# AI4REALNET/network-distributed-q-learning

Hardware: NVIDIA B200
Metric: switch_agent_decisions_per_sec (higher is better)
Workload: dtype f64

## Files before the change

### network-distributed-q-learning_b200/csrc/sfl_api.cu

```cuda
#include <stdio.h>
#include <stdlib.h>
#include <string.h>
#include <new>
#include <vector>

#include "sfl_core.cuh"

using namespace sfl;

static thread_local char g_err[512] = "";
static int fail(int code, const char *fmt, const char *detail = "") {
  snprintf(g_err, sizeof(g_err), fmt, detail);
  return code;
}

#ifndef SFL_HOST_EMUL
#include <cuda_runtime.h>
#define CU(call)                                                               \
  do {                                                                         \
    cudaError_t e_ = (call);                                                   \
    if (e_ != cudaSuccess) return fail(SFL_E_CUDA, "CUDA: %s", cudaGetErrorString(e_)); \
  } while (0)
#define CK(call)                                                               \
  do {                                                                         \
// ... 900 lines not shown
  k_shared_apply<<<c->sm_count * 8, 256, 0, (cudaStream_t)stream>>>(src, dst, d, cn, n);
  CU(cudaGetLastError());
#else
  (void)stream;
  for (size_t i = 0; i < n; i++) {
    double v = src[i];
    if (cn[i]) { v += (double)d[i] / 16777216.0 / (double)cn[i]; d[i] = 0; cn[i] = 0; }
    dst[i] = v;
  }
#endif
  return SFL_OK;
}

int sfl_shared_q_apply(void *ctx, void *stream) {
  Ctx *c = (Ctx *)ctx;
  if (!c || !c->bound) return fail(SFL_E_STATE, "sfl_bind first%s");
  DeviceGuard dg(c->device);
  if (!c->cfg.shared_q) return fail(SFL_E_STATE, "context was not created in shared-table mode%s");
  return shared_apply(c, (const double *)c->bufs.shared_q, (double *)c->bufs.shared_q, (long long *)c->bufs.shared_d, (int *)c->bufs.shared_c, stream);
}

int sfl_shared_q_apply_to(void *ctx, const void *q_src, void *q_dst, void *d, void *cnt, void *stream) {
  Ctx *c = (Ctx *)ctx;
  if (!c || !q_src || !q_dst || !d || !cnt) return fail(SFL_E_ARG, "null argument%s");
  if (!c->cfg.shared_q) return fail(SFL_E_STATE, "context was not created in shared-table mode%s");
  DeviceGuard dg(c->device);
  return shared_apply(c, (const double *)q_src, (double *)q_dst, (long long *)d, (int *)cnt, stream);
}

int sfl_total_decisions(void *ctx, uint64_t *decisions, uint64_t *ticks, void *stream) {
  Ctx *c = (Ctx *)ctx;
  if (!c || !c->bound) return fail(SFL_E_STATE, "sfl_bind first%s");
  DeviceGuard dg(c->device);
  unsigned long long out[2] = {0, 0};
#ifndef SFL_HOST_EMUL
  CK(dev_zero(c->sum_buf, 16, stream));
  k_sum<<<c->sm_count, 256, 0, (cudaStream_t)stream>>>((const sfl_env_counters *)c->bufs.counters, c->cfg.n_envs, (unsigned long long *)c->sum_buf);
  CU(cudaGetLastError());
  CK(d2h(out, c->sum_buf, 16, stream));
#else
  const sfl_env_counters *cn = (const sfl_env_counters *)c->bufs.counters;
  for (int i = 0; i < c->cfg.n_envs; i++) { out[0] += cn[i].decisions; out[1] += cn[i].ticks; }
#endif
  if (decisions) *decisions = out[0];
  if (ticks) *ticks = out[1];
  return SFL_OK;
}

int sfl_export_q(void *ctx, int env, uint32_t *keys_host, double *vals_host, int cap_rows, int *n_rows, void *stream) {
  Ctx *c = (Ctx *)ctx;
  if (!c || !c->bound) return fail(SFL_E_STATE, "sfl_bind first%s");
  DeviceGuard dg(c->device);
  if (c->cfg.eval_q) return fail(SFL_E_STATE, "an evaluation context (eval_q) keeps no per-environment tables%s");
  if (env < 0 || env >= c->cfg.n_envs || !n_rows) return fail(SFL_E_ARG, "bad env / n_rows%s");
  const Layout &L = c->L;
  size_t n = (size_t)L.q_cap * L.q_stride;
  std::vector<double> img(n);
  CK(d2h(img.data(), (char *)c->bufs.state + (size_t)env * L.env_stride + L.off_q, n * 8, stream));
  int rows = 0;
  for (int i = 0; i < L.q_cap; i++) {
    unsigned long long k;
    memcpy(&k, &img[(size_t)i * L.q_stride], 8);
    if (!k) continue;
    if (rows < cap_rows && keys_host && vals_host) {
      keys_host[rows] = (uint32_t)(k - 1);
      for (int a = 0; a < L.a_max; a++) vals_host[(size_t)rows * L.a_max + a] = img[(size_t)i * L.q_stride + 1 + a];
    }
    rows++;
  }
  *n_rows = rows;
  return rows > cap_rows && keys_host ? fail(SFL_E_NOMEM, "export buffer too small%s") : SFL_OK;
}

int sfl_import_q(void *ctx, int env, const uint32_t *keys_host, const double *vals_host, int n_rows, void *stream) {
  Ctx *c = (Ctx *)ctx;
  if (!c || !c->bound) return fail(SFL_E_STATE, "sfl_bind first%s");
  DeviceGuard dg(c->device);
  if (c->cfg.eval_q) return fail(SFL_E_STATE, "an evaluation context (eval_q) keeps no per-environment tables: use sfl_set_eval_table%s");
  if (env < 0 || env >= c->cfg.n_envs || n_rows < 0 || n_rows >= c->cfg.q_cap) return fail(SFL_E_ARG, "bad env / n_rows%s");
  const Layout &L = c->L;
  std::vector<double> img;
  int q_rows = q_image(L, keys_host, vals_host, n_rows, img);
  char *base = (char *)c->bufs.state + (size_t)env * L.env_stride;
  CK(h2d(base + L.off_q, img.data(), img.size() * 8, stream));
  CK(h2d(base + offsetof(EnvHdr, q_rows), &q_rows, 4, stream));
#ifndef SFL_HOST_EMUL
  CU(cudaStreamSynchronize((cudaStream_t)stream));
#endif
  return SFL_OK;
}

int sfl_set_eval_table(void *ctx, const uint32_t *keys_host, const double *vals_host, int n_rows, void *stream) {
  Ctx *c = (Ctx *)ctx;
  if (!c || !c->bound) return fail(SFL_E_STATE, "sfl_bind first%s");
  if (!c->cfg.eval_q) return fail(SFL_E_STATE, "the context was not created as an evaluation context (eval_q)%s");
  if (n_rows < 0 || (n_rows && (!keys_host || !vals_host))) return fail(SFL_E_ARG, "bad keys / values / n_rows%s");
  if (n_rows >= c->cfg.q_cap) {
    char detail[96];
    snprintf(detail, sizeof(detail), "%d rows, q_cap is %d", n_rows, c->cfg.q_cap);
    return fail(SFL_E_NOMEM, "the evaluation table needs q_cap above its row count (a power of two; an empty slot ends every probe): %s", detail);
  }
  DeviceGuard dg(c->device);
  std::vector<double> img;
  q_image(c->L, keys_host, vals_host, n_rows, img);
  CK(h2d(c->bufs.eval_q, img.data(), img.size() * 8, stream));
#ifndef SFL_HOST_EMUL
  CU(cudaStreamSynchronize((cudaStream_t)stream));
#endif
  return SFL_OK;
}

}
```

### network-distributed-q-learning_b200/csrc/sfl_core.cuh

```cuda
#pragma once
#include <stdint.h>
#include "switchfl_b200.h"

#if defined(__CUDACC__) && !defined(SFL_HOST_EMUL)
#define SFL_DEV 1
#define SFL_FN __device__ __forceinline__
#define SFL_NI __device__ __forceinline__
#define SFL_RARE __device__ __noinline__
#define SFL_NU _Pragma("unroll 1")
#define SFL_U4 _Pragma("unroll 4")
#define SFL_UA _Pragma("unroll")
#else
#define SFL_DEV 0
#include <math.h>
#include <string.h>
#define SFL_FN inline
#define SFL_NI inline
#define SFL_RARE inline
#define SFL_NU
#define SFL_U4
#define SFL_UA
struct int4 { int x, y, z, w; };
struct int2 { int x, y; };
static inline int4 make_int4(int x, int y, int z, int w) { int4 r = {x, y, z, w}; return r; }
// ... 47 lines not shown
};
SFL_FN int popc64(unsigned long long v) { return __builtin_popcountll(v); }
SFL_FN int ffs64(unsigned long long v) { return __builtin_ffsll((long long)v) - 1; }
SFL_FN int popc32(unsigned v) { return __builtin_popcount(v); }
SFL_FN double dmul(double a, double b) { volatile double r = a * b; return r; }
SFL_FN double dadd(double a, double b) { volatile double r = a + b; return r; }
SFL_FN double dfma(double a, double b, double c) { return fma(a, b, c); }
SFL_FN unsigned long long mulhi64(unsigned long long a, unsigned long long b) { return (unsigned long long)(((unsigned __int128)a * b) >> 64); }
template <class T> SFL_FN T ldg(const T *p) { return *p; }
#endif

template <int NW> struct TSet {
  static_assert(NW == 1 || NW == 2, "one or two words of trains");
  unsigned long long w[NW];
  SFL_FN void clear() { w[0] = 0ull; if (NW > 1) w[NW - 1] = 0ull; }
  SFL_FN void or_ballot(unsigned b, int base) {
    if (NW == 1) { w[0] |= (unsigned long long)b << base; return; }
    const unsigned long long v = (unsigned long long)b << (base & 63);
    if (base < 64) w[0] |= v; else w[NW - 1] |= v;
  }
  SFL_FN unsigned long long test(int t) const {
    if (NW == 1) return (w[0] >> t) & 1ull;
    return ((t < 64 ? w[0] : w[NW - 1]) >> (t & 63)) & 1ull;
  }
  SFL_FN int any() const { return NW == 1 ? w[0] != 0ull : (w[0] | w[NW - 1]) != 0ull; }
  SFL_FN int popc() const { return NW == 1 ? popc64(w[0]) : popc64(w[0]) + popc64(w[NW - 1]); }
  SFL_FN int pop() {
    if (NW == 1 || w[0]) { const int t = ffs64(w[0]); w[0] &= w[0] - 1; return t; }
    const int t = 64 + ffs64(w[NW - 1]); w[NW - 1] &= w[NW - 1] - 1; return t;
  }
  SFL_FN int all(int T) const {
    if (NW == 1) return w[0] == (T >= 64 ? ~0ull : ((1ull << T) - 1ull));
    return w[0] == ~0ull && w[NW - 1] == (T >= 128 ? ~0ull : ((1ull << (T - 64)) - 1ull));
  }
  SFL_FN TSet andnot(const TSet &o) const { TSet r; r.w[0] = w[0] & ~o.w[0]; if (NW > 1) r.w[NW - 1] = w[NW - 1] & ~o.w[NW - 1]; return r; }
  SFL_FN int operator==(const TSet &o) const { return NW == 1 ? w[0] == o.w[0] : (w[0] == o.w[0]) & (w[NW - 1] == o.w[NW - 1]); }
};

template <class T> struct RO {
  const T *p;
  SFL_FN T operator[](size_t i) const { return ldg(p + i); }
};

struct DevMap {
  int H, W, Hp, Wp, S, NP, NA, T, NT, max_episode_steps, a_max, pad0;
  RO<uint16_t> move;
  RO<int16_t> cell_switch;
  RO<int4> sw;
  RO<int4> port;
  RO<int4> pexit;
  RO<int4> act;
  RO<int4> train0;
  RO<int4> train1;
  RO<int> init_delay;
  RO<int> dist;
  RO<int8_t> qinit;
};

struct Layout {
  int T, S, NP, NT, a_max, q_cap, q_stride, pend_cap;
  unsigned off_tra, off_trb, off_pend, off_sem, off_rewards, off_sws, off_q;
  unsigned off_rng;
  unsigned long long env_stride;
};

struct EnvHdr {
  int elapsed, episode, step_counter, num_malf;
  int terminated, truncated, need_reset, halted;
  int err, q_rows, pending_fin, cur_dec;
  int act_cursor, ev_cursor, n_dec_logged, n_tick_logged;
  int n_ep_logged, q_init_on, aborted, cur_train;
  unsigned long long active_mask, malf_prev_mask, at_dest_mask, done_mask;
  unsigned long long decisions, ticks, train_ticks;
  double cum_reward;
  int last_next_sw;
  int eps_tag;
  unsigned eps_z, eps_w;
  unsigned long long forced_stops, stop_actions, arrived_trains;
  int dec_t, dec_go;
  unsigned long long ph[6], ph_t0;
};

struct SwS { int ninter, pad; double eps_pow; };
enum { HM_ACTIVE = 0, HM_MALF = 1, HM_DEST = 2, HM_DONE = 3 };

struct RunArgs {
  int mode, max_ticks, n_envs, trace_sem;
  int dec_cap, tick_cap, ep_cap, act_cap, ev_cap, max_steps, q_init_on, phase_clock;
  unsigned hot_bytes, env_smem, tail_hot, pad2;
  char *state;
  const sfl_hparams *hp;
  sfl_env_counters *counters;
  sfl_dec_rec *trace_dec; sfl_tick_rec *trace_tick; int4 *trace_sem_buf;
  sfl_ep_rec *ep_log; int *ep_delay;
  sfl_step_rec *step_out;
  double *sq_q; long long *sq_d; int *sq_c;
  const int8_t *replay_act; const int *replay_ev;
  const double *eval_q;
};

struct KArgs { DevMap m; Layout L; RunArgs ra; };
#define SFL_K const KArgs &K
#define c_m (K.m)
#define c_L (K.L)
#define c_ra (K.ra)

#if SFL_DEV
extern __shared__ __align__(16) char g_smem[];
typedef unsigned hot_t;
SFL_FN char *hot_ptr(hot_t o) { return g_smem + o; }
#else
typedef char *hot_t;
SFL_FN char *hot_ptr(hot_t o) { return o; }
#endif

template <bool TH, bool SQ_ = false> struct EnvT {
  static const bool SQ = SQ_;
  static const bool EVQ = false;
  static const bool HOT_TAIL = TH;
  static const int NW = 1;
  const KArgs *kp;
  hot_t hot;
  char *gb;
  SFL_FN EnvHdr *h() const { return (EnvHdr *)hot_ptr(hot); }
  SFL_FN int4 *tra() const { return (int4 *)(hot_ptr(hot) + kp->L.off_tra); }
  SFL_FN int4 *trb() const { return (int4 *)(hot_ptr(hot) + kp->L.off_trb); }
  SFL_FN char *tail() const { return TH ? hot_ptr(hot) : gb; }
  SFL_FN int2 *pend() const { return (int2 *)(tail() + kp->L.off_pend); }
  SFL_FN int4 *sem() const { return (int4 *)(tail() + kp->L.off_sem); }
  SFL_FN int *rewards() const { return (int *)(tail() + kp->L.off_rewards); }
  SFL_FN SwS *sws() const { return (SwS *)(tail() + kp->L.off_sws); }
  SFL_FN double *q() const { return (double *)(gb + kp->L.off_q); }
  hot_t own;
  SFL_FN uint8_t *own_ptr() const { return (uint8_t *)hot_ptr(own); }
  SFL_FN int owner(int p) const { return TH ? sem()[p].z : (int)(int8_t)own_ptr()[p]; }
  SFL_FN void sem_put(int p, int4 r) const { sem()[p] = r; if (!TH) own_ptr()[p] = (uint8_t)r.z; }
  SFL_FN void sem_drop(int p) const { sem()[p].z = -1; if (!TH) own_ptr()[p] = 0xFFu; }
  SFL_FN int stop_tick(int t) const { return trb()[t].w; }
  SFL_FN unsigned long long &hw0(int m) const {
    EnvHdr *x = h();
    return m == HM_ACTIVE ? x->active_mask : m == HM_MALF ? x->malf_prev_mask : m == HM_DEST ? x->at_dest_mask : x->done_mask;
  }
  SFL_FN unsigned long long *hw1(int m) const { return (unsigned long long *)(hot_ptr(hot) + sizeof(EnvHdr)) + m; }
};
template <bool TH, bool SQ_ = false> struct EnvW : EnvT<TH, SQ_> { static const int NW = 2; };
template <class Base> struct EnvEval : Base { static const bool EVQ = true; };
template <bool TH, bool SQ, int NW, bool EVQ = false> struct EnvOf { typedef EnvT<TH, SQ> type; };
template <bool TH, bool SQ> struct EnvOf<TH, SQ, 2, false> { typedef EnvW<TH, SQ> type; };
template <bool TH, int NW> struct EnvOf<TH, false, NW, true> { typedef EnvEval<typename EnvOf<TH, false, NW>::type> type; };

template <class Env> SFL_FN TSet<Env::NW> tset(const Env &e, int m) {
  TSet<Env::NW> s; s.w[0] = e.hw0(m); if (Env::NW > 1) s.w[Env::NW - 1] = *e.hw1(m); return s;
}
template <class Env> SFL_FN void tset_put(const Env &e, int m, const TSet<Env::NW> &s) { e.hw0(m) = s.w[0]; if (Env::NW > 1) *e.hw1(m) = s.w[Env::NW - 1]; }
template <class Env> SFL_FN int tset_any(const Env &e, int m) { return Env::NW == 1 ? e.hw0(m) != 0ull : (e.hw0(m) | *e.hw1(m)) != 0ull; }
template <class Env> SFL_FN int tset_pop(const Env &e, int m) { TSet<Env::NW> s = tset(e, m); const int t = s.pop(); tset_put(e, m, s); return t; }
template <class Env> SFL_FN void tset_add(const Env &e, int m, int t) {
  if (Env::NW > 1 && t >= 64) *e.hw1(m) |= 1ull << (t & 63); else e.hw0(m) |= 1ull << t;
}



struct Scratch {
  const KArgs *kp;
  hot_t base;
  SFL_FN int4 *tmp() const { return (int4 *)hot_ptr(base); }
// ... 193 lines not shown
  int n = 0, pos = SFL_MT_N;
  const unsigned rng = (unsigned)hi - (unsigned)lo;
  SFL_NU
  for (int tick = 1; hit_below && tick <= steps; tick++) {
    SFL_NU
    for (int t = 0; t < T; t++) {
      const unsigned a = mt_next(key, out, pos, g), b = mt_next(key, out, pos, g);
      if ((((unsigned long long)(a >> 5) << 26) | (b >> 6)) >= hit_below) continue;
      const int dur = lo + (int)mt_masked(key, out, pos, g, rng) + 1;
      if (g.gl == 0 && n < ev_cap) { ev[3 * n] = tick; ev[3 * n + 1] = t; ev[3 * n + 2] = dur; }
      n++;
    }
  }
  if (g.gl == 0 && n < ev_cap) ev[3 * n] = -1;
  return n;
}

struct Mv { int cell, dir, valid; };
SFL_FN unsigned mv_entry(SFL_K, int cell, int dir) { return c_m.move[(size_t)cell * 4 + dir]; }
SFL_FN int mv_valid(unsigned e, int action) { return (e >> (3 * action)) & 1; }
SFL_FN Mv mv_apply(SFL_K, unsigned e, int action, int cell) {
  unsigned f = (e >> (3 * action)) & 7u;
  int nd = (int)(f >> 1);
  int delta = (nd & 1) ? (2 - nd) : (nd - 1) * c_m.Wp;
  Mv r;
  r.cell = (e & 0x8000u) ? cell + delta : cell;
  r.dir = nd; r.valid = (int)(f & 1u);
  return r;
}
SFL_FN Mv check_action(SFL_K, int action, int cell, int dir) { return mv_apply(K, mv_entry(K, cell, dir), action, cell); }

SFL_FN int is_moving(int a) { return a >= A_LEFT && a <= A_RIGHT; }

#define SFL_NO_STOP (-0x7FFFFFFF - 1)
SFL_FN int t0_eff(int t0, int stop_tick) { return t0 > stop_tick ? t0 : stop_tick; }
template <class Env>
SFL_FN int tr_state(Env e, int t) { return (e.tra()[t].y >> 8) & 0xFF; }
template <class Env>
SFL_FN int rule_port(Env e, int port, int me, int now, int blocking_type) {
  int4 r;
  int stamp;
  if (Env::HOT_TAIL) {
    r = e.sem()[port];
    if (r.z < 0 || r.z == me) return 0;
    stamp = e.stop_tick(r.z);
  } else {
    const int holder = e.owner(port);
    if (holder < 0 || holder == me) return 0;
    r = e.sem()[port];
    stamp = e.stop_tick(holder);
  }
  if (r.x > now || t0_eff(r.x, stamp) + r.y < now) return 0;
  if (r.w == blocking_type) return 1;
  return tr_state(e, r.z) == ST_MALF;
}
template <class Env>
SFL_FN int port_blocked(Env e, int next_port, int out_port, int me, int now) {
  if (next_port >= 0) {
    if (rule_port(e, next_port, me, now, SEM_OUT)) return 1;
    return rule_port(e, out_port, me, now, SEM_IN);
  }
  return rule_port(e, out_port, me, now, SEM_OUT);
}

template <class Env>
SFL_RARE void q_insert(SFL_K, Env e, const Hp hp, unsigned key, double *row) {
  *(unsigned long long *)row = (unsigned long long)key + 1ull;
  e.h()->q_rows++;
  unsigned per_port = (unsigned)(c_L.NT * 48);
  int port = (int)(key / per_port);
  int A = c_m.sw[c_m.port[port].w].y;
  double dq = hp->default_q;
  SFL_NU
  for (int a = 0; a < A; a++) row[1 + a] = dq;
  if (c_ra.q_init_on) {
    unsigned rem = key - (unsigned)port * per_port;
    int tgt = (int)(rem / 48u), semb = (int)((rem % 48u) / 3u);
    int qi = c_m.qinit[port * c_L.NT + tgt];
    if (qi >= 0 && semb != 0) row[1 + (qi & 15)] = (qi & 16) ? 1000.0 : 500.0;
  }
}

template <class Env>
SFL_NI double *q_row(SFL_K, Env e, const Hp hp, unsigned key) {
  if (Env::SQ) return c_ra.sq_q + (size_t)key * c_L.a_max;
  unsigned mask = (unsigned)c_L.q_cap - 1u;
  unsigned i = (key * 2654435761u) >> 7;
  SFL_NU
  for (int probe = 0; probe < c_L.q_cap; probe++) {
    i &= mask;
    double *row = e.q() + (size_t)i * c_L.q_stride;
    unsigned long long k = *(unsigned long long *)row;
    if (k == (unsigned long long)key + 1ull) return row + 1;
    if (k == 0ull) {
      if (e.h()->q_rows >= c_L.q_cap - 1) break;
      q_insert(K, e, hp, key, row);
      return row + 1;
    }
    i++;
  }
  e.h()->err |= SFL_ERR_Q_FULL;
  return e.q() + 1;
}

#if SFL_DEV
SFL_FN void shared_add(long long *d, int *c, long long v) { atomicAdd((unsigned long long *)d, (unsigned long long)v); atomicAdd(c, 1); }
#else
SFL_FN void shared_add(long long *d, int *c, long long v) { *d += v; *c += 1; }
#endif

SFL_FN double lr_pow(double rate, int n) {
  double r = 1.0, b = rate;
  SFL_NU
  for (; n > 0; n >>= 1) { if (n & 1) r = dmul(r, b); b = dmul(b, b); }
  return r;
}

SFL_FN double td_value(double q, double lr, double reward, double gamma, double mq, int bootstrap) {
  const double one_m = dadd(1.0, -lr);
  return bootstrap ? dadd(dmul(one_m, q), dmul(lr, dadd(reward, dmul(gamma, mq)))) : dadd(dmul(one_m, q), dmul(lr, reward));
}

template <class Env>
SFL_NI void q_update(SFL_K, Env e, const Hp hp, unsigned key, int action, double reward,
                     const double *next_row, int prev_sw, int next_sw) {
  double *row = q_row(K, e, hp, key);
  double lr = hp->lr;
  if (hp->lr_decay_rate != 1.0) lr = dmul(lr, lr_pow(hp->lr_decay_rate, e.sws()[prev_sw].ninter));
  const double q = row[action];
  double mq = 0.0;
  if (next_sw != prev_sw && next_row) {
    int A = c_m.sw[next_sw].y;
    mq = next_row[0];
    SFL_NU
    for (int a = 1; a < A; a++) { const double v = next_row[a]; mq = v > mq ? v : mq; }
  }
  const double nq = td_value(q, lr, reward, hp->gamma, mq, next_sw != prev_sw);
  if (Env::SQ) {
    const size_t i = (size_t)key * c_L.a_max + action;
    shared_add(c_ra.sq_d + i, c_ra.sq_c + i, (long long)llrint((nq - q) * 16777216.0));
    return;
  }
  row[action] = nq;
}

template <class Row> SFL_FN int max_action_of(const Row row, int A, int mask) {
  int best = 0, b2 = -1;
  double bv = row[0], b2v = 0.0;
  if (mask & 1) { b2 = 0; b2v = bv; }
  SFL_NU
  for (int a = 1; a < A; a++) {
    const double v = row[a];
    if (v > bv) { bv = v; best = a; }
    if (((mask >> a) & 1) && (b2 < 0 || v > b2v)) { b2v = v; b2 = a; }
  }
  return ((mask >> best) & 1) ? best : b2;
}
SFL_FN int max_action(const double *row, int A, int mask) { return max_action_of(row, A, mask); }

SFL_FN int eval_action(SFL_K, unsigned key, int A, int mask) {
  const unsigned qmask = (unsigned)c_L.q_cap - 1u;
  const unsigned long long want = (unsigned long long)key + 1ull;
  unsigned i = (key * 2654435761u) >> 7;
  SFL_NU
  for (int probe = 0; probe < c_L.q_cap; probe++) {
    i &= qmask;
    const double *row = c_ra.eval_q + (size_t)i * c_L.q_stride;
    const unsigned long long k = ldg((const unsigned long long *)row);
    if (k == want) { RO<double> r; r.p = row + 1; return max_action_of(r, A, mask); }
    if (k == 0ull) break;
    i++;
  }
  return ffs64((unsigned long long)((unsigned)mask & ((1u << A) - 1u)));
}

template <class Env>
SFL_FN void sem_delete_owned(SFL_K, Env e, int port, int h) {
  int4 sw = c_m.sw[c_m.port[port].w];
  SFL_NU
  for (int k = 0; k < sw.x; k++) {
    int p = sw.z + k;
    if (e.owner(p) == h) e.sem_drop(p);
  }
}

template <class Env>
SFL_FN void transition_semaphore(SFL_K, Env e, int source, int out_port, int target, int h, int now, int st, int old_next, int old_prev) {
  if (st != ST_MALF) {
    sem_delete_owned(K, e, old_next, h);
    if (old_prev >= 0) sem_delete_owned(K, e, old_prev, h);
  }
  if (Env::HOT_TAIL) {
    int4 r = e.sem()[out_port];
    if (r.z < 0) e.sem()[out_port] = make_int4(now, 3, h, SEM_OUT);
    else if (r.w == SEM_OUT || r.x > now) e.sem()[out_port] = make_int4(now, 3, h, r.w);
    int d_ot = c_m.port[out_port].y;
    r = e.sem()[target];
    if (r.z < 0) e.sem()[target] = make_int4(now, d_ot + 1, h, SEM_IN);
    else if (r.w == SEM_IN || r.x > now) e.sem()[target] = make_int4(now, d_ot + 1, h, r.w);
    int unique = c_m.port[target].z;
    if (unique >= 0) {
      int4 up = c_m.port[unique];
      int far_port = up.x;
      if (unique != source && unique != out_port && unique != target) {
        r = e.sem()[unique];
        if (r.z < 0 || r.w == SEM_OUT || r.x > now) e.sem()[unique] = make_int4(now, d_ot + 1, h, SEM_OUT);
      }
      r = e.sem()[unique];
      if (r.z < 0 || r.x > now) e.sem()[unique] = make_int4(now, d_ot, h, SEM_OUT);
      if (far_port != source && far_port != out_port && far_port != unique) {
        r = e.sem()[far_port];
        if (r.z < 0 || r.w == SEM_IN || r.x > now) e.sem()[far_port] = make_int4(now, d_ot + up.y + 1, h, SEM_IN);
      }
    }
    if (target != source && target != out_port) {
      r = e.sem()[target];
      if (r.z < 0 || r.w == SEM_OUT || r.x > now) e.sem()[target] = make_int4(now, d_ot + 1, h, SEM_OUT);
    }
  } else {
    int4 r;
    if (e.owner(out_port) < 0) e.sem_put(out_port, make_int4(now, 3, h, SEM_OUT));
    else { r = e.sem()[out_port]; if (r.w == SEM_OUT || r.x > now) e.sem_put(out_port, make_int4(now, 3, h, r.w)); }
    int d_ot = c_m.port[out_port].y;
    if (e.owner(target) < 0) e.sem_put(target, make_int4(now, d_ot + 1, h, SEM_IN));
    else { r = e.sem()[target]; if (r.w == SEM_IN || r.x > now) e.sem_put(target, make_int4(now, d_ot + 1, h, r.w)); }
    int unique = c_m.port[target].z;
    if (unique >= 0) {
      int4 up = c_m.port[unique];
      int far_port = up.x;
      if (unique != source && unique != out_port && unique != target) {
        r = e.sem()[unique];
        if (e.owner(unique) < 0 || r.w == SEM_OUT || r.x > now) e.sem_put(unique, make_int4(now, d_ot + 1, h, SEM_OUT));
      }
      r = e.sem()[unique];
      if (e.owner(unique) < 0 || r.x > now) e.sem_put(unique, make_int4(now, d_ot, h, SEM_OUT));
      if (far_port != source && far_port != out_port && far_port != unique) {
        r = e.sem()[far_port];
        if (e.owner(far_port) < 0 || r.w == SEM_IN || r.x > now) e.sem_put(far_port, make_int4(now, d_ot + up.y + 1, h, SEM_IN));
      }
    }
    if (target != source && target != out_port) {
      r = e.sem()[target];
      if (e.owner(target) < 0 || r.w == SEM_OUT || r.x > now) e.sem_put(target, make_int4(now, d_ot + 1, h, SEM_OUT));
    }
  }
}

template <class Env>
SFL_FN int delay_at(SFL_K, Env e, int tgt_index, int cell, int dir, int now, int la) {
  int d = c_m.dist[((size_t)tgt_index * (c_m.Hp * c_m.Wp) + cell) * 4 + dir];
  if (d >= SFL_INF_DIST) { e.h()->err |= SFL_ERR_INF_DISTANCE; d = 0; }
  return now - la + d;
}

template <int KIND, class Env>
SFL_FN void finish_decision(SFL_K, Env e, const Hp hp, int env_id) {
  const bool TRACE = KIND == K_FULL;
  const int mode = run_mode<KIND>(K);
  EnvHdr *h = e.h();
  SFL_PHASE_START(h);
  if (mode == SFL_MODE_LEARN || mode == SFL_MODE_REPLAY) {
    TSet<Env::NW> fresh = tset(e, HM_DONE).andnot(tset(e, HM_DEST));
    SFL_NU
    while (fresh.any()) {
      int t = fresh.pop();
      tset_add(e, HM_DEST, t);
      int4 b = e.trb()[t];
      int n = (b.y >> 16) & 0xFF;
      SFL_NU
      for (int i = 0; i < n; i++) {
        int2 pe = e.pend()[t * c_L.pend_cap + i];
        q_update(K, e, hp, (unsigned)pe.x, (pe.y >> 24) & 15, 1000.0, nullptr, (pe.y >> 12) & 0xFFF, -1);
      }
      b.y &= 0xFFFF;
      e.trb()[t] = b;
    }
    SwS *ss = e.sws() + h->pending_fin;
    ss->ninter++;
    ss->eps_pow = dmul(ss->eps_pow, hp->epsilon_decay_rate);
  }
  h->pending_fin = -1;
  SFL_PHASE_MARK(h, PH_UPDATE);
  if (h->step_counter > c_ra.max_steps) h->truncated = 1;
  if (TRACE) {
    if (c_ra.trace_dec && h->cur_dec >= 0 && h->cur_dec < c_ra.dec_cap) {
      sfl_dec_rec *rec = c_ra.trace_dec + (size_t)env_id * c_ra.dec_cap + h->cur_dec;
      rec->arrived = h->done_mask; rec->arrived_hi = Env::NW > 1 ? *e.hw1(HM_DONE) : 0ull;
      rec->done = h->terminated | (h->truncated << 1);
      if (c_ra.trace_sem_buf) {
        int4 *dst = c_ra.trace_sem_buf + ((size_t)env_id * c_ra.dec_cap + h->cur_dec) * c_L.NP;
        SFL_NU
        for (int p = 0; p < c_L.NP; p++) {
          int4 r = e.sem()[p];
          if (r.z >= 0) r.x = t0_eff(r.x, e.stop_tick(r.z));
          r.y += r.x; dst[p] = r;
        }
      }
    }
    h->cur_dec = -1;
  }
}

template <int G, class Env>
SFL_FN int observe_bits(SFL_K, Env e, const Grp<G> &g, const int on, const int t) {
  const int now = e.h()->elapsed;
  const int s = on ? (e.trb()[t].y & 0xFFFF) : 0;
  const int4 sw = c_m.sw[s];
  unsigned bits = 0;
  SFL_UA
  for (int base = 0; base < 8; base += G) {
    const int j = base + g.gl;
    int b = 0;
    if (on && j < 8 && (j & 3) < sw.x) {
      const int port = sw.z + (j & 3);
      b = (j & 4) ? rule_port(e, port, t, now, SEM_IN) : rule_port(e, c_m.port[port].x, t, now, SEM_OUT);
    }
    bits |= (g.ballot(b) & 0xFFu) << base;
  }
  return (int)(~(bits | (bits >> 4)) & ((1u << sw.x) - 1u));
}

struct Obs { int s, P, A, p0, a0, cur, semb, mask, ok; unsigned key; };
template <class Env>
SFL_FN Obs observe(SFL_K, Env e, int t, int now, const int4 ta, const int4 tb, const int semb_pre = -1) {
  Obs ob;
  ob.s = tb.y & 0xFFFF;
  const int4 sw = c_m.sw[ob.s];
  ob.P = sw.x; ob.A = sw.y; ob.p0 = sw.z; ob.a0 = sw.w;
  const int4 tr0 = c_m.train0[t], tr1 = c_m.train1[t];
  const int my_port = (int)((unsigned)ta.w >> 16);
  const int dist_now = c_m.dist[((size_t)tr0.w * (c_m.Hp * c_m.Wp) + ta.x) * 4 + (ta.y & 0xFF)];
  int semb = semb_pre;
  if (semb_pre < 0) {
    semb = 0;
    SFL_NU
    for (int k = 0; k < ob.P; k++)
      if (!port_blocked(e, c_m.port[ob.p0 + k].x, ob.p0 + k, t, now)) semb |= 1 << k;
  }
  ob.semb = semb;
  ob.cur = my_port - ob.p0;
  ob.ok = ob.cur >= 0 && ob.cur < ob.P;
  ob.key = 0u; ob.mask = 0;
  if (!ob.ok) return ob;
  int delay = now - tr1.y + dist_now;
  if (dist_now >= SFL_INF_DIST) { e.h()->err |= SFL_ERR_INF_DISTANCE; delay = now - tr1.y; }
  int level = delay <= 0 ? 0 : (delay <= (tr1.y - tr1.x) * 20 ? 1 : 2);
  ob.key = (((unsigned)(ob.p0 + ob.cur) * c_L.NT + tr0.w) * 16u + semb) * 3u + level;
  const int4 px = c_m.pexit[ob.p0 + ob.cur];
  int mask = 1 << (ob.A - 1);
  {
    int ex[3] = {px.y, px.z, px.w};
#if SFL_DEV
#pragma unroll
#endif
    for (int i = 0; i < 3; i++) if (i < px.x && ((semb >> ((ex[i] >> 4) & 3)) & 1)) mask |= 1 << (ex[i] & 15);
  }
  ob.mask = mask;
  return ob;
}

template <int KIND, class Env>
SFL_FN void decide(SFL_K, Env e, const Hp hp, int env_id, int t, const int semb_pre = -1) {
  const bool TRACE = KIND == K_FULL;
  const int mode = run_mode<KIND>(K);
  EnvHdr *h = e.h();
  const int now = h->elapsed;
  SFL_PHASE_START(h);
  int4 ta = e.tra()[t], tb = e.trb()[t];
  const int learning = mode == SFL_MODE_LEARN || mode == SFL_MODE_REPLAY;
  const int s_early = tb.y & 0xFFFF;
  const int reward_in = e.rewards()[s_early * c_L.T + t];
  double eps_pow = 1.0;
  int ninter = 0;
  if (mode == SFL_MODE_LEARN) {
    eps_pow = e.sws()[s_early].eps_pow;
    if (KIND == K_FULL && c_L.off_rng) ninter = e.sws()[s_early].ninter;
  }
  int2 pend0 = make_int2(0, -1);
  if (learning && ((tb.y >> 16) & 0xFF)) pend0 = e.pend()[t * c_L.pend_cap];
  const Obs ob = observe(K, e, t, now, ta, tb, semb_pre);
  if (!ob.ok) {
    h->err |= SFL_ERR_NO_TRAIN_AT_SWITCH; h->aborted++; h->truncated = 1;
    return;
  }
  const int s = ob.s, A = ob.A, p0 = ob.p0, a0 = ob.a0, cur = ob.cur, mask = ob.mask;
  const unsigned key = ob.key;
  const int4 tr0 = c_m.train0[t], tr1 = c_m.train1[t];
  const int pos = ta.x, dir = ta.y & 0xFF, st = (ta.y >> 8) & 0xFF;
  const int my_port = (int)((unsigned)ta.w >> 16);
  SFL_PHASE_MARK(h, PH_OBSERVE);
  double *my_row = nullptr;
  int action = -1;
  if (mode == SFL_MODE_REPLAY || mode == SFL_MODE_STEP) {
    if (mode == SFL_MODE_STEP) h->act_cursor = 0;
    int exploited = 0;
    if (h->act_cursor >= c_ra.act_cap) { h->err |= SFL_ERR_REPLAY_UNDERRUN; action = A - 1; }
    else {
      action = c_ra.replay_act[(size_t)env_id * c_ra.act_cap + h->act_cursor++];
      if (mode == SFL_MODE_REPLAY && action >= 0 && (action & 0x40)) { exploited = 1; action &= 0x3F; }
    }
    if (action < 0 || action >= A) { h->err |= SFL_ERR_BAD_ACTION; action = A - 1; }
    if (exploited) {
      my_row = q_row(K, e, hp, key);
      if (max_action(my_row, A, mask) != action) h->err |= SFL_ERR_REPLAY_DIVERGED;
    }
  } else if (KIND == K_FULL && mode == SFL_MODE_LEARN && c_L.off_rng) {
    Pcg *gp = (Pcg *)(hot_ptr(e.hot) + c_L.off_rng);
    Pcg g = *gp;
    if (eps_explore(pcg_double(g), hp->epsilon, hp->epsilon_decay_rate, ninter, eps_pow)) action = pcg_explore_action(g, mask);
    *gp = g;
  } else if (mode == SFL_MODE_LEARN) {
    double eps = dmul(hp->epsilon, eps_pow);
    const int pair = h->step_counter >> 1;
    unsigned ux, uy;
    if ((h->step_counter & 1) && h->eps_tag == pair) { ux = h->eps_z; uy = h->eps_w; }
    else {
      const U4 u = philox4x32((unsigned)pair, (unsigned)(hp->episode_base + h->episode), 0x5F1u, 0u, (unsigned)hp->seed, (unsigned)(hp->seed >> 32));
      h->eps_tag = pair; h->eps_z = u.z; h->eps_w = u.w;
      if (h->step_counter & 1) { ux = u.z; uy = u.w; } else { ux = u.x; uy = u.y; }
    }
    double u01 = ((double)ux + 0.5) * (1.0 / 4294967296.0);
    if (u01 < eps) {
      int pick = (int)(((unsigned long long)uy * (unsigned)popc32((unsigned)mask)) >> 32);
      unsigned mm = (unsigned)mask;
      SFL_NU
      for (; pick > 0; pick--) mm &= mm - 1;
      action = ffs64(mm);
    }
  }
  if (action < 0) {
    if (Env::EVQ) action = eval_action(K, key, A, mask);
    else {
      my_row = q_row(K, e, hp, key);
      action = max_action(my_row, A, mask);
    }
  }
  SFL_PHASE_MARK(h, PH_ACT);
  int moving = 0, move2 = A_STOP, in_port = my_port, out_port = my_port;
  if (action != A - 1) {
    int4 ac = c_m.act[a0 + action];
    if (ac.x == cur) { moving = 1; move2 = ac.z; in_port = p0 + ac.x; out_port = p0 + ac.y; }
  }
  int next_switch = s, next_port = -1;
  if (moving) {
    int4 op = c_m.port[out_port];
    next_port = op.x;
    int old_prev = (tb.x & 0xFFFF) == 0xFFFF ? -1 : (tb.x & 0xFFFF);
    transition_semaphore(K, e, in_port, out_port, next_port, t, now, st, my_port, old_prev);
    tb.x = (out_port & 0xFFFF) | (in_port << 16);
    ta.w = (ta.w & 0xFFFF) | (next_port << 16);
    next_switch = c_m.port[next_port].w;
  }
  unsigned plan = (unsigned)ta.z & 0xFFFFu;
  int pl = ta.z >> 16;
  if (moving && pl > 0) { plan = (plan & 0xFu) | ((unsigned)move2 << 4); pl = 2; }
  else if (!moving) {
    if (pl >= SFL_PLAN_CAP) { h->err |= SFL_ERR_PLAN_FULL; pl = SFL_PLAN_CAP - 1; }
    plan = ((plan << 4) | A_STOP) & 0xFFFFu; pl++;
  } else { plan = A_FWD | ((unsigned)move2 << 4); pl = 2; }
  ta.z = (int)plan | (pl << 16);
  e.tra()[t] = ta;
  int all_blocked = 1;
  if ((plan & 0xFu) == A_STOP) {
    if (moving) all_blocked = port_blocked(e, next_port, out_port, t, now);
    else all_blocked = (mask == (1 << (A - 1)));
  }
  int cell = pos, d2 = dir;
  {
    unsigned pp = plan;
    SFL_NU
    for (int i = 0; i < pl; i++, pp >>= 4) {
      int a = pp & 0xF;
      if (a != A_STOP) { Mv c = check_action(K, a, cell, d2); cell = c.cell; d2 = c.dir; }
    }
  }
  int curr = delay_at(K, e, tr0.w, cell, d2, now, tr1.y);
  int reward_out = tb.z - curr;
  if (!all_blocked && (plan & 0xFu) == A_STOP) reward_out -= 1300;
  e.rewards()[next_switch * c_L.T + t] = reward_out;
  tb.z = curr;
  h->step_counter++;
  SFL_PHASE_MARK(h, PH_APPLY);
  if (learning) {
    int n = (tb.y >> 16) & 0xFF;
    int2 *pend = e.pend() + t * c_L.pend_cap;
    int hit = -1, same = -1;
    SFL_NU
    for (int i = 0; i < n; i++) {
      int nsw = (i ? pend[i].y : pend0.y) & 0xFFF;
      if (nsw == s && hit < 0) hit = i;
    }
    if (hit >= 0) {
      int2 pe = hit ? pend[hit] : pend0;
      const int prev_sw = (pe.y >> 12) & 0xFFF;
      if (prev_sw != s && !my_row) my_row = q_row(K, e, hp, key);
      q_update(K, e, hp, (unsigned)pe.x, (pe.y >> 24) & 15, (double)reward_in, my_row, prev_sw, s);
      SFL_NU
      for (int j = hit; j + 1 < n; j++) pend[j] = pend[j + 1];
      n--;
    }
    int meta = next_switch | (s << 12) | (action << 24);
    SFL_NU
    for (int i = 0; i < n; i++) if ((pend[i].y & 0xFFF) == next_switch) same = i;
    if (same >= 0) pend[same] = make_int2((int)key, meta);
    else if (n >= c_L.pend_cap) h->err |= SFL_ERR_PEND_FULL;
    else { pend[n] = make_int2((int)key, meta); n++; }
    tb.y = (tb.y & 0xFFFF) | (n << 16);
  }
  e.trb()[t] = tb;
  SFL_PHASE_MARK(h, PH_UPDATE);
  h->cum_reward += (double)reward_in;
  if (TRACE) {
    if (c_ra.trace_dec) {
      h->cur_dec = h->n_dec_logged;
      if (h->n_dec_logged < c_ra.dec_cap) {
        sfl_dec_rec *rec = c_ra.trace_dec + (size_t)env_id * c_ra.dec_cap + h->n_dec_logged;
        rec->ep = h->episode; rec->tick = now; rec->sw = s; rec->train = t; rec->key = key; rec->mask = mask;
        rec->action = action; rec->next_sw = next_switch; rec->reward = reward_in; rec->done = 0; rec->arrived = 0;
        rec->arrived_hi = 0;
      }
      h->n_dec_logged++;
    }
  }
  if (TRACE) h->last_next_sw = next_switch;
  h->decisions++;
  if (mask == (1 << (A - 1))) h->forced_stops++;
  if (action == A - 1) h->stop_actions++;
  h->pending_fin = s;
}

template <int G, class Env>
SFL_RARE void env_reset(SFL_K, Env e, const Grp<G> &g, int on) {
  EnvHdr *h = e.h();
  const int T = on ? c_L.T : 0, NP = on ? c_L.NP : 0;
  SFL_NU
  for (int t = g.gl; t < T; t += G) {
    int4 tr0 = c_m.train0[t], tr1 = c_m.train1[t];
    e.tra()[t] = make_int4(-1, tr0.y | (ST_WAITING << 8) | (0 << 16) | (A_NONE << 24), 0, (int)((unsigned)tr1.z << 16));
    int4 b = e.trb()[t];
    e.trb()[t] = make_int4(b.x, 0xFFFF, c_m.init_delay[t], SFL_NO_STOP);
  }
  SFL_NU
  for (int p = g.gl; p < NP; p += G) e.sem_put(p, make_int4(0, 0, -1, 0));
  SFL_NU
  for (int i = g.gl; i < c_L.S * T; i += G) e.rewards()[i] = 0;
  g.sync();
  if (on && g.gl == 0) {
    SFL_NU
    for (int t = 0; t < T; t++) {
      int4 tr1 = c_m.train1[t];
      e.sem_put(tr1.z, make_int4(tr1.x - 2, tr1.w + 2, t, SEM_IN));
    }
    h->elapsed = 0; h->step_counter = 0; h->num_malf = 0; h->terminated = 0; h->truncated = 0; h->need_reset = 0;
    h->pending_fin = -1; h->cur_dec = -1; h->ev_cursor = 0; h->active_mask = 0; h->malf_prev_mask = 0; h->at_dest_mask = 0;
    h->eps_tag = -1;
    h->done_mask = 0; h->cum_reward = 0.0;
    if (Env::NW > 1) { SFL_UA for (int m = 0; m < 4; m++) *e.hw1(m) = 0ull; }
  }
  g.sync();
}

template <int NW> struct TickRegs {
  int elapsed, ended, rng_blk;
  TSet<NW> active, done;
  unsigned ticks, train_ticks;
};

SFL_FN int malf_stage2(const Hp hp, int now, int t) {
  const U4 u = philox4x32((unsigned)now, (unsigned)t, 0xA11Eu, 0u, (unsigned)hp->seed, (unsigned)(hp->seed >> 32));
  if (u.x >= hp->malf_thr2) return 0;
  return hp->malf_min + (int)(((unsigned long long)u.y * (unsigned)(hp->malf_max - hp->malf_min + 1)) >> 32) + 1;
}

template <int G, int KIND, bool ONE, class Env>
SFL_FN void env_tick(SFL_K, Env e, Scratch sc, const Hp hp, int env_id, const Grp<G> &g, TickRegs<Env::NW> &R, const int live) {
  const bool TRACE = KIND == K_FULL;
  EnvHdr *h = e.h();
  const int Tw = c_L.T;
  const int T = live ? Tw : 0;
  const int now = R.elapsed + 1;
  const int replay_ev = KIND != K_LEARN && c_ra.replay_ev != 0;
  const unsigned thr = live ? hp->malf_threshold : 0u;
  if (replay_ev) {
    SFL_NU
    for (int t = g.gl; t < T; t += G) sc.inj()[t] = 0;
    g.sync();
    if (live && g.gl == 0) {
      const int *ev = c_ra.replay_ev + (size_t)env_id * c_ra.ev_cap * 3;
      int c = h->ev_cursor;
// ... 402 lines not shown
```

Measured before the change: 425.1 million.

## Cache Q-table slot indices in pending updates to skip hash re-probing

Pending TD updates now store the Q-table slot index, tagged with a flag bit, in place of the raw key whenever the slot is known. The later update can then address the row directly instead of re-running the hash probe. The first two pending entries are prefetched with a single vector load, the hit's Q value is read early, and hit-removal and same-switch search are merged into one compaction pass. Importing a Q table now converts tagged entries back to keys on the host, because a rebuilt table invalidates the stored slots. This adds some host-side transfers on import.

```diff
diff --git a/network-distributed-q-learning_b200/csrc/sfl_api.cu b/network-distributed-q-learning_b200/csrc/sfl_api.cu
--- a/network-distributed-q-learning_b200/csrc/sfl_api.cu
+++ b/network-distributed-q-learning_b200/csrc/sfl_api.cu
@@ -1006,6 +1006,23 @@
   std::vector<double> img;
   int q_rows = q_image(L, keys_host, vals_host, n_rows, img);
   char *base = (char *)c->bufs.state + (size_t)env * L.env_stride;
+  std::vector<int4> trb(L.T);
+  std::vector<int2> pend((size_t)L.T * L.pend_cap);
+  CK(d2h(trb.data(), base + L.off_trb, trb.size() * sizeof(int4), stream));
+  CK(d2h(pend.data(), base + L.off_pend, pend.size() * sizeof(int2), stream));
+  int untagged = 0;
+  for (int t = 0; t < L.T; t++) {
+    const int n = (trb[t].y >> 16) & 0xFF;
+    for (int i = 0; i < n; i++) {
+      int2 &pe = pend[(size_t)t * L.pend_cap + i];
+      if (!(pe.y & SFL_PEND_SLOT)) continue;
+      unsigned long long k = 0;
+      CK(d2h(&k, base + L.off_q + (size_t)pe.x * L.q_stride * 8, 8, stream));
+      pe.x = (int)(unsigned)(k - 1ull); pe.y &= ~SFL_PEND_SLOT;
+      untagged++;
+    }
+  }
+  if (untagged) CK(h2d(base + L.off_pend, pend.data(), pend.size() * sizeof(int2), stream));
   CK(h2d(base + L.off_q, img.data(), img.size() * 8, stream));
   CK(h2d(base + offsetof(EnvHdr, q_rows), &q_rows, 4, stream));
 #ifndef SFL_HOST_EMUL
diff --git a/network-distributed-q-learning_b200/csrc/sfl_core.cuh b/network-distributed-q-learning_b200/csrc/sfl_core.cuh
--- a/network-distributed-q-learning_b200/csrc/sfl_core.cuh
+++ b/network-distributed-q-learning_b200/csrc/sfl_core.cuh
@@ -153,6 +153,7 @@
 };
 
 struct SwS { int ninter, pad; double eps_pow; };
+#define SFL_PEND_SLOT (1 << 28)
 enum { HM_ACTIVE = 0, HM_MALF = 1, HM_DEST = 2, HM_DONE = 3 };
 
 struct RunArgs {
@@ -512,7 +513,8 @@
 }
 
 template <class Env>
-SFL_NI double *q_row(SFL_K, Env e, const Hp hp, unsigned key) {
+SFL_NI double *q_row(SFL_K, Env e, const Hp hp, unsigned key, int &slot) {
+  slot = -1;
   if (Env::SQ) return c_ra.sq_q + (size_t)key * c_L.a_max;
   unsigned mask = (unsigned)c_L.q_cap - 1u;
   unsigned i = (key * 2654435761u) >> 7;
@@ -521,16 +523,25 @@
     i &= mask;
     double *row = e.q() + (size_t)i * c_L.q_stride;
     unsigned long long k = *(unsigned long long *)row;
-    if (k == (unsigned long long)key + 1ull) return row + 1;
+    if (k == (unsigned long long)key + 1ull) { slot = (int)i; return row + 1; }
     if (k == 0ull) {
       if (e.h()->q_rows >= c_L.q_cap - 1) break;
       q_insert(K, e, hp, key, row);
+      slot = (int)i;
       return row + 1;
     }
     i++;
   }
   e.h()->err |= SFL_ERR_Q_FULL;
   return e.q() + 1;
+}
+template <class Env>
+SFL_NI double *q_row(SFL_K, Env e, const Hp hp, unsigned key) { int slot; return q_row(K, e, hp, key, slot); }
+template <class Env>
+SFL_FN double *q_slot(SFL_K, Env e, int slot) { return e.q() + (size_t)slot * c_L.q_stride + 1; }
+template <class Env>
+SFL_NI double *pend_row(SFL_K, Env e, const Hp hp, int2 pe) {
+  return !Env::SQ && (pe.y & SFL_PEND_SLOT) ? q_slot(K, e, pe.x) : q_row(K, e, hp, (unsigned)pe.x);
 }
 
 #if SFL_DEV
@@ -552,12 +563,10 @@
 }
 
 template <class Env>
-SFL_NI void q_update(SFL_K, Env e, const Hp hp, unsigned key, int action, double reward,
+SFL_NI void q_update(SFL_K, Env e, const Hp hp, double *row, unsigned key, int action, double q, double reward,
                      const double *next_row, int prev_sw, int next_sw) {
-  double *row = q_row(K, e, hp, key);
   double lr = hp->lr;
   if (hp->lr_decay_rate != 1.0) lr = dmul(lr, lr_pow(hp->lr_decay_rate, e.sws()[prev_sw].ninter));
-  const double q = row[action];
   double mq = 0.0;
   if (next_sw != prev_sw && next_row) {
     int A = c_m.sw[next_sw].y;
@@ -699,8 +708,10 @@
       int n = (b.y >> 16) & 0xFF;
       SFL_NU
       for (int i = 0; i < n; i++) {
-        int2 pe = e.pend()[t * c_L.pend_cap + i];
-        q_update(K, e, hp, (unsigned)pe.x, (pe.y >> 24) & 15, 1000.0, nullptr, (pe.y >> 12) & 0xFFF, -1);
+        const int2 pe = e.pend()[t * c_L.pend_cap + i];
+        const int a = (pe.y >> 24) & 15;
+        double *row = pend_row(K, e, hp, pe);
+        q_update(K, e, hp, row, (unsigned)pe.x, a, row[a], 1000.0, nullptr, (pe.y >> 12) & 0xFFF, -1);
       }
       b.y &= 0xFFFF;
       e.trb()[t] = b;
@@ -806,8 +817,13 @@
     eps_pow = e.sws()[s_early].eps_pow;
     if (KIND == K_FULL && c_L.off_rng) ninter = e.sws()[s_early].ninter;
   }
-  int2 pend0 = make_int2(0, -1);
-  if (learning && ((tb.y >> 16) & 0xFF)) pend0 = e.pend()[t * c_L.pend_cap];
+  const int n_pend = learning ? (tb.y >> 16) & 0xFF : 0;
+  int2 *pend = e.pend() + t * c_L.pend_cap;
+  int2 pend0 = make_int2(0, -1), pend1 = make_int2(0, -1);
+  if (n_pend) {
+    if (c_L.pend_cap & 1) { pend0 = pend[0]; if (n_pend > 1) pend1 = pend[1]; }
+    else { const int4 v = *(const int4 *)pend; pend0 = make_int2(v.x, v.y); pend1 = make_int2(v.z, v.w); }
+  }
   const Obs ob = observe(K, e, t, now, ta, tb, semb_pre);
   if (!ob.ok) {
     h->err |= SFL_ERR_NO_TRAIN_AT_SWITCH; h->aborted++; h->truncated = 1;
@@ -820,6 +836,7 @@
   const int my_port = (int)((unsigned)ta.w >> 16);
   SFL_PHASE_MARK(h, PH_OBSERVE);
   double *my_row = nullptr;
+  int my_slot = -1;
   int action = -1;
   if (mode == SFL_MODE_REPLAY || mode == SFL_MODE_STEP) {
     if (mode == SFL_MODE_STEP) h->act_cursor = 0;
@@ -831,7 +848,7 @@
     }
     if (action < 0 || action >= A) { h->err |= SFL_ERR_BAD_ACTION; action = A - 1; }
     if (exploited) {
-      my_row = q_row(K, e, hp, key);
+      my_row = q_row(K, e, hp, key, my_slot);
       if (max_action(my_row, A, mask) != action) h->err |= SFL_ERR_REPLAY_DIVERGED;
     }
   } else if (KIND == K_FULL && mode == SFL_MODE_LEARN && c_L.off_rng) {
@@ -861,8 +878,17 @@
   if (action < 0) {
     if (Env::EVQ) action = eval_action(K, key, A, mask);
     else {
-      my_row = q_row(K, e, hp, key);
+      my_row = q_row(K, e, hp, key, my_slot);
       action = max_action(my_row, A, mask);
+    }
+  }
+  double q_hit = 0.0;
+  int q_hit_ok = 0;
+  if (!Env::SQ && n_pend && my_row) {
+    const int2 pe = (pend0.y & 0xFFF) == s ? pend0 : pend1;
+    if (((pend0.y & 0xFFF) == s || (n_pend > 1 && (pend1.y & 0xFFF) == s)) && (pe.y & SFL_PEND_SLOT)) {
+      q_hit = q_slot(K, e, pe.x)[(pe.y >> 24) & 15];
+      q_hit_ok = 1;
     }
   }
   SFL_PHASE_MARK(h, PH_ACT);
@@ -912,29 +938,34 @@
   h->step_counter++;
   SFL_PHASE_MARK(h, PH_APPLY);
   if (learning) {
-    int n = (tb.y >> 16) & 0xFF;
-    int2 *pend = e.pend() + t * c_L.pend_cap;
-    int hit = -1, same = -1;
+    int hit = -1, same = -1, n = 0;
+    int2 hit_e = make_int2(0, 0);
     SFL_NU
-    for (int i = 0; i < n; i++) {
-      int nsw = (i ? pend[i].y : pend0.y) & 0xFFF;
-      if (nsw == s && hit < 0) hit = i;
+    for (int i = 0; i < n_pend; i++) {
+      int2 pe;
+      if (i == 0) pe = pend0;
+      else if (i == 1) pe = pend1;
+      else pe = pend[i];
+      if (hit < 0 && (pe.y & 0xFFF) == s) { hit = i; hit_e = pe; continue; }
+      if ((pe.y & 0xFFF) == next_switch) same = n;
+      if (n != i) pend[n] = pe;
+      n++;
     }
     if (hit >= 0) {
-      int2 pe = hit ? pend[hit] : pend0;
-      const int prev_sw = (pe.y >> 12) & 0xFFF;
-      if (prev_sw != s && !my_row) my_row = q_row(K, e, hp, key);
-      q_update(K, e, hp, (unsigned)pe.x, (pe.y >> 24) & 15, (double)reward_in, my_row, prev_sw, s);
-      SFL_NU
-      for (int j = hit; j + 1 < n; j++) pend[j] = pend[j + 1];
-      n--;
-    }
-    int meta = next_switch | (s << 12) | (action << 24);
-    SFL_NU
-    for (int i = 0; i < n; i++) if ((pend[i].y & 0xFFF) == next_switch) same = i;
-    if (same >= 0) pend[same] = make_int2((int)key, meta);
+      const int prev_sw = (hit_e.y >> 12) & 0xFFF, a = (hit_e.y >> 24) & 15;
+      const int tagged = !Env::SQ && (hit_e.y & SFL_PEND_SLOT);
+      double *row = nullptr;
+      double q = 0.0;
+      if (tagged) { row = q_slot(K, e, hit_e.x); q = q_hit_ok ? q_hit : row[a]; }
+      if (prev_sw != s && !my_row) my_row = q_row(K, e, hp, key, my_slot);
+      if (!tagged) { row = q_row(K, e, hp, (unsigned)hit_e.x); q = row[a]; }
+      q_update(K, e, hp, row, (unsigned)hit_e.x, a, q, (double)reward_in, my_row, prev_sw, s);
+    }
+    const int2 ne = my_slot >= 0 ? make_int2(my_slot, next_switch | (s << 12) | (action << 24) | SFL_PEND_SLOT)
+                                 : make_int2((int)key, next_switch | (s << 12) | (action << 24));
+    if (same >= 0) pend[same] = ne;
     else if (n >= c_L.pend_cap) h->err |= SFL_ERR_PEND_FULL;
-    else { pend[n] = make_int2((int)key, meta); n++; }
+    else { pend[n] = ne; n++; }
     tb.y = (tb.y & 0xFFFF) | (n << 16);
   }
   e.trb()[t] = tb;
```

New measurement: 391.1 million (median of 6 runs). 0.92x the previous value.
